# ziwang1121/IEEE

Measured on AMD Instinct MI355X. Metric: 3-modal images/s (train fwd+bwd), higher is better.
Workload: dtype bf16

## Files before the change

ieee_amd/csrc/bn.hip:

```cpp
#include <math.h>
#include <stdlib.h>

#include <hip/hip_ext.h>

#include <algorithm>
#include "common.h"
#include "pool_gather.h"

namespace ieee {

#ifndef IEEE_RED_MAX_BLOCKS
#define IEEE_RED_MAX_BLOCKS 768
#endif
constexpr int RED_MAX_BLOCKS = IEEE_RED_MAX_BLOCKS;

struct RedGeom {
  int M, C;
  int cprw;
  int tx, ty;
  int cblocks;
  int rblocks;
  int rows_per_block;
};

static RedGeom red_geom(int64_t M, int C, int vec) {
  RedGeom g;
  g.M = (int)M;
  g.C = C;
  g.cprw = C / vec;
  g.tx = g.cprw < 64 ? g.cprw : 64;
  int tx = 1;
  while (tx * 2 <= g.tx && g.cprw % (tx * 2) == 0) tx *= 2;
  g.tx = tx;
  g.ty = 256 / g.tx;
  g.cblocks = cdiv(g.cprw, g.tx);
  int rb = RED_MAX_BLOCKS / g.cblocks;
  if (rb < 1) rb = 1;
  const int maxrb = cdiv(M, g.ty * 4);
  if (rb > maxrb) rb = maxrb;
  if (rb < 1) rb = 1;
  g.rows_per_block = cdiv(cdiv(M, rb), g.ty) * g.ty;
  g.rblocks = cdiv(M, g.rows_per_block);
  return g;
}

template <typename T, int NQ, class F>
__device__ __forceinline__ void reduce_channels(const RedGeom& g, float* partial, int64_t partial_gs, F f) {
  constexpr int VEC = 16 / sizeof(T);
  __shared__ float red[256 * 8];
  const int t = threadIdx.x;
  const int tx = t % g.tx, ty = t / g.tx;
  const int cb = blockIdx.x % g.cblocks, rb = blockIdx.x / g.cblocks;
  const int chunk = cb * g.tx + tx;
  float acc[NQ][VEC];
#pragma unroll
  for (int q = 0; q < NQ; ++q)
#pragma unroll
    for (int e = 0; e < VEC; ++e) acc[q][e] = 0.f;
// ... 675 lines not shown
#pragma unroll
    for (int e = 0; e < VEC; ++e) {
      const float m = (v[e] * sc[c0 + e] + sh[c0 + e]) > 0.f ? d[e] : 0.f;
      acc[0][e] += m;
      acc[1][e] += m * v[e];
    }
  });
}

template <typename T>
__global__ __launch_bounds__(256) void bn_bwd_pooled_apply_kernel(const T* __restrict__ dpool,
                                                                  const uint8_t* __restrict__ arg,
                                                                  const T* __restrict__ y, T* __restrict__ dy,
                                                                  const float* __restrict__ coef, int64_t coef_gs,
                                                                  int64_t total_chunks, int cprw, int C, int64_t y_gs,
                                                                  int64_t p_gs, int Hi, int Wi, int Ho, int Wo,
                                                                  const float* __restrict__ stats, int64_t stats_gs,
                                                                  PoolShifts ps) {
  constexpr int VEC = 16 / sizeof(T);
  const int z = blockIdx.y;
  const float* sc = stats + z * stats_gs + 2 * C;
  const float* sh = sc + C;
  const float* k1 = coef + z * coef_gs;
  const float* k2 = k1 + C;
  const float* k3 = k2 + C;
  const T* dd = dpool + z * p_gs;
  const uint8_t* aa = arg + z * p_gs;
  const T* yy = y + z * y_gs;
  T* oo = dy + z * y_gs;
  const uint32_t total = (uint32_t)total_chunks, stride = gridDim.x * blockDim.x;
  for (uint32_t i = blockIdx.x * blockDim.x + threadIdx.x; i < total; i += stride) {
    int ch, row, w, h, b;
    if (ps.pow2) {
      ch = (int)(i & (uint32_t)(cprw - 1)); row = (int)(i >> ps.lq);
      w = row & (Wi - 1); h = (row >> ps.lw) & (Hi - 1); b = row >> (ps.lw + ps.lh);
    } else {
      ch = (int)(i % (uint32_t)cprw); row = (int)(i / (uint32_t)cprw);
      w = row % Wi; h = (row / Wi) % Hi; b = row / (Wi * Hi);
    }
    const int c0 = ch * VEC;
    float d[VEC], v[VEC];
    const uint4 yv = *(const uint4*)(yy + (int64_t)i * VEC);
    pool_grad_gather<T>(dd, aa, b, h, w, ch, Ho, Wo, C, d);
    Vec16<T>::unpack(yv, v);
#pragma unroll
    for (int e = 0; e < VEC; ++e) {
      const float m = (v[e] * sc[c0 + e] + sh[c0 + e]) > 0.f ? d[e] : 0.f;
      v[e] = k1[c0 + e] * m + k2[c0 + e] * v[e] + k3[c0 + e];
    }
    *(uint4*)(oo + (int64_t)i * VEC) = Vec16<T>::pack(v);
  }
}

template <typename T, bool APPLY>
__global__ __launch_bounds__(256) void bn_bwd_pooled_tiled_kernel(const T* __restrict__ dpool, const uint8_t* __restrict__ arg,
                                                                  const T* __restrict__ y, T* __restrict__ dy,
                                                                  const float* __restrict__ coef, int64_t coef_gs,
                                                                  float* __restrict__ partial, int64_t partial_gs, int C,
                                                                  int64_t y_gs, int64_t p_gs, int Hi, int Wi, int Ho, int Wo,
                                                                  const float* __restrict__ stats, int64_t stats_gs) {
  constexpr int VEC = 16 / sizeof(T);
  extern __shared__ __attribute__((aligned(16))) char pooled_lds[];
  const int z = blockIdx.y, t = threadIdx.x;
  const int hp = Hi >> 1;
  const int b = blockIdx.x / hp, p = blockIdx.x - b * hp;
  const int cprw = C / VEC, rowel = Wo * C;
  T* sd = (T*)pooled_lds;
  uint8_t* sa = (uint8_t*)(pooled_lds + 2 * rowel * sizeof(T));
  const bool has2 = p + 1 < Ho;
  {
    const int64_t o = z * p_gs + ((int64_t)b * Ho + p) * rowel;
    const uint4* dsrc = (const uint4*)(dpool + o);
    const uint4* asrc = (const uint4*)(arg + o);
    const int nd = (has2 ? 2 : 1) * rowel / VEC, na = (has2 ? 2 : 1) * rowel / 16;
    for (int i = t; i < nd; i += 256) ((uint4*)sd)[i] = dsrc[i];
    for (int i = t; i < na; i += 256) ((uint4*)sa)[i] = asrc[i];
  }
  __syncthreads();
  const float* sc = stats + z * stats_gs + 2 * C;
  const float* sh = sc + C;
  const float* k1 = coef + z * coef_gs;
  const float* k2 = k1 + C;
  const float* k3 = k2 + C;
  const T* yy = y + z * y_gs + (int64_t)b * Hi * Wi * C;
  T* oo = APPLY ? dy + z * y_gs + (int64_t)b * Hi * Wi * C : nullptr;
  const int ch = t % cprw, c0 = ch * VEC;
  float scl[VEC], shf[VEC], a1[VEC], a2[VEC], a3[VEC];
#pragma unroll
  for (int e = 0; e < VEC; ++e) {
    scl[e] = sc[c0 + e]; shf[e] = sh[c0 + e];
    if (APPLY) { a1[e] = k1[c0 + e]; a2[e] = k2[c0 + e]; a3[e] = k3[c0 + e]; } else { a1[e] = 0.f; a2[e] = 0.f; a3[e] = 0.f; }
  }
  float s1[VEC], s2[VEC];
#pragma unroll
  for (int e = 0; e < VEC; ++e) { s1[e] = 0.f; s2[e] = 0.f; }
  const int ppr = 256 / cprw;
  for (int px = t / cprw; px < 2 * Wi; px += ppr) {
    const int r = px >= Wi ? 1 : 0, w = px - r * Wi;
    const int q0 = w >> 1, lr0 = r + 1, lc0 = (w & 1) + 1;
    const bool c1 = (w & 1) && q0 + 1 < Wo, r1 = r == 1 && has2;
    const int64_t off = ((int64_t)(2 * p + r) * Wi + w) * C + c0;
    const uint4 yv = *(const uint4*)(yy + off);
    float d[VEC];
#pragma unroll
    for (int e = 0; e < VEC; ++e) d[e] = 0.f;
    auto window = [&](int lrow, int q, int local) {
      const int o = (lrow * Wo + q) * C + c0;
      float g[VEC];
      Vec16<T>::unpack(*(const uint4*)(sd + o), g);
      if constexpr (VEC == 8) {
        const uint2 av = *(const uint2*)(sa + o);
#pragma unroll
        for (int e = 0; e < 4; ++e) {
          if ((int)((av.x >> (8 * e)) & 0xff) == local) d[e] += g[e];
          if ((int)((av.y >> (8 * e)) & 0xff) == local) d[4 + e] += g[4 + e];
        }
      } else {
        const uint32_t av = *(const uint32_t*)(sa + o);
#pragma unroll
        for (int e = 0; e < VEC; ++e)
          if ((int)((av >> (8 * e)) & 0xff) == local) d[e] += g[e];
      }
    };
    window(0, q0, lr0 * 3 + lc0);
    if (c1) window(0, q0 + 1, lr0 * 3);
    if (r1) window(1, q0, lc0);
    if (r1 && c1) window(1, q0 + 1, 0);
    float v[VEC];
    Vec16<T>::unpack(yv, v);
#pragma unroll
    for (int e = 0; e < VEC; ++e) {
      const float m = (v[e] * scl[e] + shf[e]) > 0.f ? d[e] : 0.f;
      if (APPLY) {
        v[e] = a1[e] * m + a2[e] * v[e] + a3[e];
      } else {
        s1[e] += m;
        s2[e] += m * v[e];
      }
    }
    if (APPLY) *(uint4*)(oo + off) = Vec16<T>::pack(v);
  }
  if constexpr (!APPLY) {
    float* red = (float*)pooled_lds;
    float* out = partial + z * partial_gs + (int64_t)blockIdx.x * 2 * C;
#pragma unroll
    for (int qn = 0; qn < 2; ++qn) {
      __syncthreads();
#pragma unroll
      for (int e = 0; e < VEC; ++e) red[t * VEC + e] = qn == 0 ? s1[e] : s2[e];
      __syncthreads();
      for (int c = t; c < C; c += 256) {
        const int cc = c / VEC, e = c - cc * VEC;
        float s = 0.f;
        for (int k = cc; k < 256; k += cprw) s += red[k * VEC + e];
        out[qn * C + c] = s;
      }
    }
  }
}

static int tot_blocks(int64_t chunks, int64_t groups) {
  static const int64_t fixed = getenv("IEEE_BN_TOTALS_BLOCKS") ? atoll(getenv("IEEE_BN_TOTALS_BLOCKS")) : 0;
  const int64_t cap = fixed > 0 ? fixed : std::max<int64_t>(256, 2048 / std::max<int64_t>(groups, 1));
  int64_t b = (chunks + 255) / 256;
  if (b > cap) b = cap;
  if (b < 1) b = 1;
  return (int)b;
}

static int ew_blocks(int64_t chunks) {
  static const int64_t cap = getenv("IEEE_EW_BLOCKS") ? atoll(getenv("IEEE_EW_BLOCKS")) : 8192;
  int64_t b = (chunks + 255) / 256;
  if (b > cap) b = cap;
  if (b < 1) b = 1;
  return (int)b;
}

}

using namespace ieee;

static int vec_of(int dtype) { return dtype == IEEE_BF16 ? 8 : 4; }

static bool fixed_channel_ok(int which, int cprw, const void* p1, const void* p2) {
  static const int on = getenv("IEEE_BN_FIXED") ? atoi(getenv("IEEE_BN_FIXED")) : 8;
  return (on & which) && cprw >= 1 && cprw <= 256 && 256 % cprw == 0 && ((uintptr_t)p1 & 15) == 0 && ((uintptr_t)p2 & 15) == 0;
}
static int fixed_unroll() {
  static const int u = getenv("IEEE_BN_UNROLL") ? atoi(getenv("IEEE_BN_UNROLL")) : 1;
  return u == 2 ? 2 : 1;
}

extern "C" int64_t ieee_bn_partial_floats(int dtype, int64_t M, int64_t C) {
  const RedGeom g = red_geom(M, (int)C, vec_of(dtype));
  const int64_t rb = std::max((int64_t)g.rblocks, (M + 127) / 128);
  return rb * 2 * C;
}

extern "C" int ieee_bn2d_fwd(const void* y, const void* residual, void* out, int dtype, int64_t groups, int64_t M,
                             int64_t C, int64_t act_gs, const float* gamma, const float* beta, int64_t param_gs,
                             float* running_mean, float* running_var, int64_t buf_gs, float* stats, float* partial,
                             float momentum, float eps, int training, int relu, int64_t stats_rblocks, void* relu_bits,
                             void* stream) {
  IEEE_REQUIRE(y && gamma && beta && stats, "bn2d_fwd: null pointer");
  IEEE_REQUIRE(!relu_bits || (dtype == IEEE_BF16 && out && act_gs % 8 == 0), "bn2d_fwd: relu_bits needs a bf16 output");
  IEEE_REQUIRE(dtype == IEEE_F32 || dtype == IEEE_BF16, "bn2d_fwd: bad dtype");
  IEEE_REQUIRE(C % vec_of(dtype) == 0, "bn2d_fwd: C %ld not a multiple of %d", (long)C, vec_of(dtype));
  IEEE_REQUIRE(training || (running_mean && running_var), "bn2d_fwd: eval mode needs running stats");
  IEEE_REQUIRE(!training || partial, "bn2d_fwd: training needs the partial-sum scratch");
  hipStream_t st = (hipStream_t)stream;
  RedGeom g = red_geom(M, (int)C, vec_of(dtype));
// ... 252 lines not shown
                          (const bf16*)dout, (const bf16*)out_mask, (const bf16*)y, (bf16*)dy, (bf16*)g_out,                 \
                          (const long long*)totals, gamma, param_gs, stats, dgamma, dbeta, grad_gs, (int)M, chunks, cprw,    \
                          (int)C, act_gs, 1.0 / (double)M, replicas, groups * 2 * C, overflow);                              \
    break;
  switch (variant) {
    IEEE_BN_BWD_TOT(0, false) IEEE_BN_BWD_TOT(0, true) IEEE_BN_BWD_TOT(1, false) IEEE_BN_BWD_TOT(1, true)
    IEEE_BN_BWD_TOT(2, false) IEEE_BN_BWD_TOT(2, true)
  }
#undef IEEE_BN_BWD_TOT
  return launch_status("bn_bwd_apply_totals_kernel");
}

extern "C" int ieee_bn2d_bwd_totals_ds(const void* dout, const void* y, const void* y_ds, void* dy, int dtype, int64_t groups,
                                       int64_t M, int64_t C, int64_t act_gs, const float* gamma, int64_t param_gs,
                                       const float* stats, float* dgamma, float* dbeta, int64_t grad_gs, const void* totals,
                                       int replicas, void* totals_ds, int replicas_ds, int* overflow, void* done_event,
                                       void* stream) {
  IEEE_REQUIRE(replicas >= 1 && replicas <= 64 && replicas_ds >= 1 && replicas_ds <= 64, "bn2d_bwd_totals_ds: 1..64 replicas");
  IEEE_REQUIRE(dout && y && y_ds && dy && gamma && stats && totals && totals_ds, "bn2d_bwd_totals_ds: null pointer");
  IEEE_REQUIRE(dtype == IEEE_BF16, "bn2d_bwd_totals_ds: bf16 only");
  const int cprw = (int)(C / 8);
  IEEE_REQUIRE(C % 8 == 0 && cprw >= 1 && cprw <= 256 && 256 % cprw == 0, "bn2d_bwd_totals_ds: C / 8 must divide 256");
  IEEE_REQUIRE((((uintptr_t)totals | (uintptr_t)gamma | (uintptr_t)stats) & 15) == 0 && param_gs % 4 == 0,
               "bn2d_bwd_totals_ds: totals / gamma / stats must be 16-byte aligned (group stride a multiple of 4 floats)");
  hipStream_t st = (hipStream_t)stream;
  const int64_t chunks = M * C / 8;
  dim3 grid(tot_blocks(chunks, groups), (unsigned)groups);
  const size_t lds = std::max<size_t>(3 * C, 8 * 256) * sizeof(float);
  const float lim2 = nextafterf(4611686018427387904.0f / (float)grid.x, 0.f);
  hipExtLaunchKernelGGL((bn_bwd_apply_totals_ds_kernel<bf16>), grid, dim3(256), (uint32_t)lds, st, nullptr, (hipEvent_t)done_event, 0,
                        (const bf16*)dout, (const bf16*)y, (const bf16*)y_ds, (bf16*)dy, (const long long*)totals, gamma, param_gs,
                        stats, dgamma, dbeta, grad_gs, (int)M, chunks, cprw, (int)C, act_gs, 1.0 / (double)M, replicas,
                        groups * 2 * C, (long long*)totals_ds, replicas_ds, groups * 2 * C, lim2, overflow);
  return launch_status("bn_bwd_apply_totals_ds_kernel");
}

extern "C" int ieee_bn2d_bwd_pooled(const void* dpool, const uint8_t* argmax, const void* y, void* dy, int dtype,
                                    int64_t groups, int64_t B, int64_t Hi, int64_t Wi, int64_t C, const float* gamma,
                                    int64_t param_gs, const float* stats, float* dgamma, float* dbeta, int64_t grad_gs,
                                    float* partial, float* coef, int accumulate, void* stream) {
  IEEE_REQUIRE(dpool && argmax && y && dy && gamma && stats && partial && coef, "bn2d_bwd_pooled: null pointer");
  IEEE_REQUIRE(dtype == IEEE_F32 || dtype == IEEE_BF16, "bn2d_bwd_pooled: bad dtype");
  IEEE_REQUIRE(C % vec_of(dtype) == 0, "bn2d_bwd_pooled: C not a multiple of the vector width");
  IEEE_REQUIRE(B * Hi * Wi * C < (1ll << 31), "bn2d_bwd_pooled: more than 2^31 elements per group");
  hipStream_t st = (hipStream_t)stream;
  const int64_t M = B * Hi * Wi;
  const int Ho = (int)((Hi + 2 - 3) / 2 + 1), Wo = (int)((Wi + 2 - 3) / 2 + 1);
  const int64_t y_gs = M * C, p_gs = B * Ho * Wo * C;
  RedGeom g = red_geom(M, (int)C, vec_of(dtype));
  {
    static const bool tiled_on = !(getenv("IEEE_POOLED_TILED") && atoi(getenv("IEEE_POOLED_TILED")) == 0);
    const int vec = vec_of(dtype), es = dtype == IEEE_BF16 ? 2 : 4;
    const int64_t cprw = C / vec, rowel = (int64_t)Wo * C;
    const int64_t lds = std::max<int64_t>(2 * rowel * (es + 1), 256 * vec * 4);
    const int64_t rbt = B * (Hi / 2);
    if (tiled_on && Hi == 2 * Ho && Wi == 2 * Wo && Wi >= 64 && 256 % cprw == 0 && rowel % 16 == 0 && lds <= 64 * 1024 &&
        rbt <= (M + 127) / 128) {
      const int64_t partial_gs = rbt * 2 * C;
      dim3 tgrid((unsigned)rbt, (unsigned)groups);
      if (dtype == IEEE_F32)
        bn_bwd_pooled_tiled_kernel<float, false><<<tgrid, 256, lds, st>>>((const float*)dpool, argmax, (const float*)y, nullptr,
            coef, 3 * C, partial, partial_gs, (int)C, y_gs, p_gs, (int)Hi, (int)Wi, Ho, Wo, stats, 4 * C);
      else
        bn_bwd_pooled_tiled_kernel<bf16, false><<<tgrid, 256, lds, st>>>((const bf16*)dpool, argmax, (const bf16*)y, nullptr,
            coef, 3 * C, partial, partial_gs, (int)C, y_gs, p_gs, (int)Hi, (int)Wi, Ho, Wo, stats, 4 * C);
      IEEE_TRY(launch_status("bn_bwd_pooled_tiled_kernel(reduce)"));
      const int lpc = finalize_lpc(rbt);
      bn_bwd_finalize_kernel<<<dim3(cdiv(C, 256 / lpc), (unsigned)groups), 256, 0, st>>>(
          partial, partial_gs, (int)rbt, (int)M, (int)C, gamma, param_gs, stats, 4 * C, dgamma, dbeta, grad_gs, coef, 3 * C,
          accumulate, 0, lpc);
      IEEE_TRY(launch_status("bn_bwd_finalize_kernel"));
      if (dtype == IEEE_F32)
        bn_bwd_pooled_tiled_kernel<float, true><<<tgrid, 256, lds, st>>>((const float*)dpool, argmax, (const float*)y, (float*)dy,
            coef, 3 * C, nullptr, 0, (int)C, y_gs, p_gs, (int)Hi, (int)Wi, Ho, Wo, stats, 4 * C);
      else
        bn_bwd_pooled_tiled_kernel<bf16, true><<<tgrid, 256, lds, st>>>((const bf16*)dpool, argmax, (const bf16*)y, (bf16*)dy,
            coef, 3 * C, nullptr, 0, (int)C, y_gs, p_gs, (int)Hi, (int)Wi, Ho, Wo, stats, 4 * C);
      return launch_status("bn_bwd_pooled_tiled_kernel(apply)");
    }
  }
  const int64_t partial_gs = (int64_t)g.rblocks * 2 * C;
  dim3 rgrid(g.cblocks * g.rblocks, (unsigned)groups);
  auto lg = [](int64_t v) { int l = 0; while ((1ll << l) < v) ++l; return ((1ll << l) == v) ? l : -1; };
  PoolShifts ps;
  ps.lw = lg(Wi); ps.lh = lg(Hi); ps.lc = lg(C); ps.lq = lg(g.cprw);
  ps.pow2 = (ps.lw >= 0 && ps.lh >= 0 && ps.lc >= 0 && ps.lq >= 0) ? 1 : 0;
  if (dtype == IEEE_F32)
    bn_bwd_pooled_reduce_kernel<float><<<rgrid, 256, 0, st>>>((const float*)dpool, argmax, (const float*)y, y_gs, p_gs, g,
                                                              (int)Hi, (int)Wi, Ho, Wo, partial, partial_gs, stats, 4 * C, ps);
  else
    bn_bwd_pooled_reduce_kernel<bf16><<<rgrid, 256, 0, st>>>((const bf16*)dpool, argmax, (const bf16*)y, y_gs, p_gs, g,
                                                             (int)Hi, (int)Wi, Ho, Wo, partial, partial_gs, stats, 4 * C, ps);
  IEEE_TRY(launch_status("bn_bwd_pooled_reduce_kernel"));
  const int lpc = finalize_lpc(g.rblocks);
  bn_bwd_finalize_kernel<<<dim3(cdiv(C, 256 / lpc), (unsigned)groups), 256, 0, st>>>(
      partial, partial_gs, g.rblocks, (int)M, (int)C, gamma, param_gs, stats, 4 * C, dgamma, dbeta, grad_gs, coef,
      3 * C, accumulate, 0, lpc);
  IEEE_TRY(launch_status("bn_bwd_finalize_kernel"));
  const int64_t chunks = M * C / vec_of(dtype);
  dim3 grid(ew_blocks(chunks), (unsigned)groups);
  if (dtype == IEEE_F32)
    bn_bwd_pooled_apply_kernel<float><<<grid, 256, 0, st>>>((const float*)dpool, argmax, (const float*)y, (float*)dy, coef,
                                                            3 * C, chunks, g.cprw, (int)C, y_gs, p_gs, (int)Hi, (int)Wi, Ho,
                                                            Wo, stats, 4 * C, ps);
  else
    bn_bwd_pooled_apply_kernel<bf16><<<grid, 256, 0, st>>>((const bf16*)dpool, argmax, (const bf16*)y, (bf16*)dy, coef,
                                                           3 * C, chunks, g.cprw, (int)C, y_gs, p_gs, (int)Hi, (int)Wi, Ho,
                                                           Wo, stats, 4 * C, ps);
  return launch_status("bn_bwd_pooled_apply_kernel");
}
```

ieee_amd/csrc/cim.hip:

```cpp
#include <stdlib.h>

#include <type_traits>

#include "common.h"
#include "pool_gather.h"

namespace ieee {

template <typename T>
__global__ void nchw_to_nhwc_kernel(const float* x0, const float* x1, const float* x2, T* out, int B, int C, int H,
                                    int W, int Cpad, int pad) {
  const int z = blockIdx.y;
  const float* x = z == 0 ? x0 : (z == 1 ? x1 : x2);
  const int Hp = H + 2 * pad, Wp = W + 2 * pad;
  const int64_t total = (int64_t)B * Hp * Wp * Cpad;
  T* o = out + z * total;
  for (int64_t i = (int64_t)blockIdx.x * blockDim.x + threadIdx.x; i < total; i += (int64_t)gridDim.x * blockDim.x) {
    const int c = (int)(i % Cpad);
    int64_t p = i / Cpad;
    const int wp = (int)(p % Wp); p /= Wp;
    const int hp = (int)(p % Hp);
    const int b = (int)(p / Hp);
    const int h = hp - pad, w = wp - pad;
    float v = 0.f;
// ... 44 lines not shown
  out += z * o_gs;
  arg += z * o_gs;
  for (int i = blockIdx.x * blockDim.x + threadIdx.x; i < total; i += gridDim.x * blockDim.x) {
    int ch, q, pp, b;
    if (lq >= 0) {
      ch = i & (cprw - 1);
      const int p = i >> lq;
      q = p & (Wo - 1); pp = (p >> lw) & (Ho - 1); b = p >> (lw + lh);
    } else {
      ch = i % cprw;
      int p = i / cprw;
      q = p % Wo; p /= Wo;
      pp = p % Ho;
      b = p / Ho;
    }
    float best[VEC];
    int bi[VEC];
#pragma unroll
    for (int e = 0; e < VEC; ++e) { best[e] = -INFINITY; bi[e] = 0; }
#pragma unroll
    for (int r = 0; r < 3; ++r) {
      const int h = pp * 2 - 1 + r;
      if ((unsigned)h >= (unsigned)Hi) continue;
#pragma unroll
      for (int s = 0; s < 3; ++s) {
        const int w = q * 2 - 1 + s;
        if ((unsigned)w >= (unsigned)Wi) continue;
        float v[VEC];
        Vec16<T>::unpack(*(const uint4*)(x + (((int64_t)b * Hi + h) * Wi + w) * C + ch * VEC), v);
        if constexpr (AFFINE) {
#pragma unroll
          for (int e = 0; e < VEC; ++e) v[e] = fmaxf(v[e] * sc[ch * VEC + e] + sh[ch * VEC + e], 0.f);
          Vec16<T>::unpack(Vec16<T>::pack(v), v);
        }
#pragma unroll
        for (int e = 0; e < VEC; ++e)
          if (v[e] > best[e]) { best[e] = v[e]; bi[e] = r * 3 + s; }
      }
    }
    const int64_t o = (((int64_t)b * Ho + pp) * Wo + q) * C + ch * VEC;
    *(uint4*)(out + o) = Vec16<T>::pack(best);
    if constexpr (VEC == 8) {
      uint2 pk = make_uint2(0u, 0u);
#pragma unroll
      for (int e = 0; e < 4; ++e) { pk.x |= (unsigned)bi[e] << (8 * e); pk.y |= (unsigned)bi[4 + e] << (8 * e); }
      *(uint2*)(arg + o) = pk;
    } else {
#pragma unroll
      for (int e = 0; e < VEC; ++e) arg[o + e] = (uint8_t)bi[e];
    }
  }
}

template <typename T>
__global__ __launch_bounds__(256) void bn_relu_maxpool_tiled_kernel(const T* __restrict__ y, T* __restrict__ out,
                                                                    uint8_t* __restrict__ arg, int Hi, int Wi, int C, int Ho,
                                                                    int Wo, int64_t x_gs, int64_t o_gs,
                                                                    const float* __restrict__ stats, int64_t stats_gs) {
  constexpr int VEC = 16 / sizeof(T);
  extern __shared__ __attribute__((aligned(16))) char pool_lds[];
  T* sa = (T*)pool_lds;
  const int z = blockIdx.y, t = threadIdx.x;
  const int b = blockIdx.x / Ho, p = blockIdx.x - b * Ho;
  const int cprw = C / VEC, rowch = Wi * cprw;
  const float* sc = stats + z * stats_gs + 2 * C;
  const float* sh = sc + C;
  const T* yy = y + z * x_gs + (int64_t)b * Hi * Wi * C;
  for (int idx = t; idx < 3 * rowch; idx += 256) {
    const int r = idx / rowch, rem = idx - r * rowch;
    const int h = 2 * p - 1 + r;
    if ((unsigned)h >= (unsigned)Hi) continue;
    const int c0 = (rem % cprw) * VEC;
    float v[VEC];
    Vec16<T>::unpack(*(const uint4*)(yy + ((int64_t)h * Wi) * C + (int64_t)rem * VEC), v);
#pragma unroll
    for (int e = 0; e < VEC; ++e) v[e] = fmaxf(v[e] * sc[c0 + e] + sh[c0 + e], 0.f);
    *(uint4*)(sa + (int64_t)idx * VEC) = Vec16<T>::pack(v);
  }
  __syncthreads();
  for (int idx = t; idx < Wo * cprw; idx += 256) {
    const int q = idx / cprw, ch = idx - q * cprw;
    float best[VEC];
    int bi[VEC];
#pragma unroll
    for (int e = 0; e < VEC; ++e) { best[e] = -INFINITY; bi[e] = 0; }
#pragma unroll
    for (int r = 0; r < 3; ++r) {
      const int h = 2 * p - 1 + r;
      if ((unsigned)h >= (unsigned)Hi) continue;
#pragma unroll
      for (int s2 = 0; s2 < 3; ++s2) {
        const int w = q * 2 - 1 + s2;
        if ((unsigned)w >= (unsigned)Wi) continue;
        float v[VEC];
        Vec16<T>::unpack(*(const uint4*)(sa + ((int64_t)(r * Wi + w) * cprw + ch) * VEC), v);
#pragma unroll
        for (int e = 0; e < VEC; ++e)
          if (v[e] > best[e]) { best[e] = v[e]; bi[e] = r * 3 + s2; }
      }
    }
    const int64_t o = z * o_gs + (((int64_t)b * Ho + p) * Wo + q) * C + ch * VEC;
    *(uint4*)(out + o) = Vec16<T>::pack(best);
    if constexpr (VEC == 8) {
      uint2 pk = make_uint2(0u, 0u);
#pragma unroll
      for (int e = 0; e < 4; ++e) { pk.x |= (unsigned)bi[e] << (8 * e); pk.y |= (unsigned)bi[4 + e] << (8 * e); }
      *(uint2*)(arg + o) = pk;
    } else {
#pragma unroll
      for (int e = 0; e < VEC; ++e) arg[o + e] = (uint8_t)bi[e];
    }
  }
}

template <typename T>
__global__ __launch_bounds__(256) void maxpool_bwd_kernel(const T* __restrict__ dout, const uint8_t* __restrict__ arg,
                                                          T* __restrict__ dx, int B, int Hi, int Wi, int C, int Ho,
                                                          int Wo, int64_t x_gs, int64_t o_gs) {
  constexpr int VEC = 16 / sizeof(T);
  const int z = blockIdx.y;
  const int cprw = C / VEC;
  const int total = B * Hi * Wi * cprw;
  dout += z * o_gs;
  arg += z * o_gs;
  dx += z * x_gs;
  for (int i = blockIdx.x * blockDim.x + threadIdx.x; i < total; i += gridDim.x * blockDim.x) {
    const int ch = i % cprw;
    int p = i / cprw;
    const int w = p % Wi; p /= Wi;
    const int h = p % Hi;
    const int b = p / Hi;
    float acc[VEC];
    pool_grad_gather<T>(dout, arg, b, h, w, ch, Ho, Wo, C, acc);
    *(uint4*)(dx + i * VEC) = Vec16<T>::pack(acc);
  }
}

struct PosGeom {
  int B, P, C;
  int W;
  int cprw, tx, ty, cblocks;
};
static PosGeom pos_geom(int B, int H, int W, int C, int vec) {
  PosGeom g;
  g.B = B; g.P = H * W; g.C = C; g.W = W;
  g.cprw = C / vec;
  int tx = 1;
  while (tx * 2 <= 64 && g.cprw % (tx * 2) == 0) tx *= 2;
  g.tx = tx;
  g.ty = 256 / tx;
  g.cblocks = g.cprw / tx;
  return g;
}

__device__ __forceinline__ int bin_start(int i, int H, int parts) { return (i * H) / parts; }
__device__ __forceinline__ int bin_end(int i, int H, int parts) { return ((i + 1) * H + parts - 1) / parts; }

constexpr int RED_Q = 8;
template <int NQV>
__device__ __forceinline__ void reduce_over_ty(float* acc, int tx, int ty, int txn, int tyn, float* red) {
#pragma unroll
  for (int q0 = 0; q0 < NQV; q0 += RED_Q) {
    __syncthreads();
#pragma unroll
    for (int q = 0; q < RED_Q; ++q)
// ... 469 lines not shown
  do {                                                              \
    if ((dtype) == IEEE_F32) { CALL_F32; }                          \
    else if ((dtype) == IEEE_BF16) { CALL_BF16; }                   \
    else { IEEE_REQUIRE(false, "bad dtype %d", (int)(dtype)); }     \
  } while (0)

extern "C" int ieee_nchw_to_nhwc3(const float* x_rgb, const float* x_ni, const float* x_ti, void* out, int dtype,
                                  int64_t B, int64_t C, int64_t H, int64_t W, int64_t Cpad, int64_t pad, void* stream) {
  IEEE_REQUIRE(x_rgb && x_ni && x_ti && out, "nchw_to_nhwc3: null pointer");
  IEEE_REQUIRE(Cpad >= C && pad >= 0, "nchw_to_nhwc3: Cpad < C or negative padding");
  hipStream_t st = (hipStream_t)stream;
  if (dtype == IEEE_BF16 && Cpad == 4 && C <= 4 && ((W + 2 * pad) & 1) == 0 &&
      B * (H + 2 * pad) * (W + 2 * pad) < (1ll << 30)) {
    dim3 grid2(ew_blocks2(B * (H + 2 * pad) * ((W + 2 * pad) / 2)), 3);
    nchw_to_nhwc4_bf16_kernel<<<grid2, 256, 0, st>>>(x_rgb, x_ni, x_ti, (bf16*)out, (int)B, (int)C, (int)H, (int)W, (int)pad);
    return launch_status("nchw_to_nhwc4_bf16_kernel");
  }
  dim3 grid(ew_blocks2(B * Cpad * (H + 2 * pad) * (W + 2 * pad)), 3);
  DISPATCH_T(dtype, (nchw_to_nhwc_kernel<float><<<grid, 256, 0, st>>>(x_rgb, x_ni, x_ti, (float*)out, (int)B, (int)C, (int)H, (int)W, (int)Cpad, (int)pad)),
             (nchw_to_nhwc_kernel<bf16><<<grid, 256, 0, st>>>(x_rgb, x_ni, x_ti, (bf16*)out, (int)B, (int)C, (int)H, (int)W, (int)Cpad, (int)pad)));
  return launch_status("nchw_to_nhwc_kernel");
}

extern "C" int ieee_maxpool3x3s2_fwd(const void* x, void* out, uint8_t* argmax, int dtype, int64_t groups, int64_t B,
                                     int64_t Hi, int64_t Wi, int64_t C, void* stream) {
  IEEE_REQUIRE(x && out && argmax, "maxpool_fwd: null pointer");
  IEEE_REQUIRE(C % vecw(dtype) == 0, "maxpool_fwd: C not a multiple of the vector width");
  IEEE_REQUIRE(B * Hi * Wi * C < (1ll << 31), "maxpool_fwd: more than 2^31 elements per group");
  const int Ho = (int)((Hi + 2 - 3) / 2 + 1), Wo = (int)((Wi + 2 - 3) / 2 + 1);
  hipStream_t st = (hipStream_t)stream;
  dim3 grid(ew_blocks2(B * Ho * Wo * C / vecw(dtype)), (unsigned)groups);
  const int64_t xgs = B * Hi * Wi * C, ogs = B * Ho * Wo * C;
  auto lg = [](int64_t v) { int l = 0; while ((1ll << l) < v) ++l; return ((1ll << l) == v) ? l : -1; };
  int lq = lg(C / vecw(dtype)), lw = lg(Wo), lh = lg(Ho);
  if (lq < 0 || lw < 0 || lh < 0) lq = -1;
  DISPATCH_T(dtype, (maxpool_fwd_kernel<float, false><<<grid, 256, 0, st>>>((const float*)x, (float*)out, argmax, (int)B, (int)Hi, (int)Wi, (int)C, Ho, Wo, xgs, ogs, lq, lw, lh, nullptr, 0)),
             (maxpool_fwd_kernel<bf16, false><<<grid, 256, 0, st>>>((const bf16*)x, (bf16*)out, argmax, (int)B, (int)Hi, (int)Wi, (int)C, Ho, Wo, xgs, ogs, lq, lw, lh, nullptr, 0)));
  return launch_status("maxpool_fwd_kernel");
}

extern "C" int ieee_bn_relu_maxpool3x3s2_fwd(const void* y, const float* stats, void* out, uint8_t* argmax, int dtype,
                                             int64_t groups, int64_t B, int64_t Hi, int64_t Wi, int64_t C, void* stream) {
  IEEE_REQUIRE(y && stats && out && argmax, "bn_relu_maxpool_fwd: null pointer");
  IEEE_REQUIRE(C % vecw(dtype) == 0, "bn_relu_maxpool_fwd: C not a multiple of the vector width");
  IEEE_REQUIRE(B * Hi * Wi * C < (1ll << 31), "bn_relu_maxpool_fwd: more than 2^31 elements per group");
  const int Ho = (int)((Hi + 2 - 3) / 2 + 1), Wo = (int)((Wi + 2 - 3) / 2 + 1);
  hipStream_t st = (hipStream_t)stream;
  dim3 grid(ew_blocks2(B * Ho * Wo * C / vecw(dtype)), (unsigned)groups);
  const int64_t xgs = B * Hi * Wi * C, ogs = B * Ho * Wo * C;
  {
    static const bool tiled_on = !(getenv("IEEE_POOL_TILED") && atoi(getenv("IEEE_POOL_TILED")) == 0);
    const int64_t lds = 3 * Wi * C * (dtype == IEEE_BF16 ? 2 : 4);
    if (tiled_on && lds <= 64 * 1024 && Wi >= 32) {
      dim3 tgrid((unsigned)(B * Ho), (unsigned)groups);
      DISPATCH_T(dtype, (bn_relu_maxpool_tiled_kernel<float><<<tgrid, 256, lds, st>>>((const float*)y, (float*)out, argmax, (int)Hi, (int)Wi, (int)C, Ho, Wo, xgs, ogs, stats, 4 * C)),
                 (bn_relu_maxpool_tiled_kernel<bf16><<<tgrid, 256, lds, st>>>((const bf16*)y, (bf16*)out, argmax, (int)Hi, (int)Wi, (int)C, Ho, Wo, xgs, ogs, stats, 4 * C)));
      return launch_status("bn_relu_maxpool_tiled_kernel");
    }
  }
  auto lg = [](int64_t v) { int l = 0; while ((1ll << l) < v) ++l; return ((1ll << l) == v) ? l : -1; };
  int lq = lg(C / vecw(dtype)), lw = lg(Wo), lh = lg(Ho);
  if (lq < 0 || lw < 0 || lh < 0) lq = -1;
  DISPATCH_T(dtype, (maxpool_fwd_kernel<float, true><<<grid, 256, 0, st>>>((const float*)y, (float*)out, argmax, (int)B, (int)Hi, (int)Wi, (int)C, Ho, Wo, xgs, ogs, lq, lw, lh, stats, 4 * C)),
             (maxpool_fwd_kernel<bf16, true><<<grid, 256, 0, st>>>((const bf16*)y, (bf16*)out, argmax, (int)B, (int)Hi, (int)Wi, (int)C, Ho, Wo, xgs, ogs, lq, lw, lh, stats, 4 * C)));
  return launch_status("maxpool_fwd_kernel(affine)");
}

extern "C" int ieee_maxpool3x3s2_bwd(const void* dout, const uint8_t* argmax, void* dx, int dtype, int64_t groups,
                                     int64_t B, int64_t Hi, int64_t Wi, int64_t C, void* stream) {
  IEEE_REQUIRE(dout && dx && argmax, "maxpool_bwd: null pointer");
  IEEE_REQUIRE(B * Hi * Wi * C < (1ll << 31), "maxpool_bwd: more than 2^31 elements per group");
  const int Ho = (int)((Hi + 2 - 3) / 2 + 1), Wo = (int)((Wi + 2 - 3) / 2 + 1);
  hipStream_t st = (hipStream_t)stream;
  dim3 grid(ew_blocks2(B * Hi * Wi * C / vecw(dtype)), (unsigned)groups);
  const int64_t xgs = B * Hi * Wi * C, ogs = B * Ho * Wo * C;
  DISPATCH_T(dtype, (maxpool_bwd_kernel<float><<<grid, 256, 0, st>>>((const float*)dout, argmax, (float*)dx, (int)B, (int)Hi, (int)Wi, (int)C, Ho, Wo, xgs, ogs)),
             (maxpool_bwd_kernel<bf16><<<grid, 256, 0, st>>>((const bf16*)dout, argmax, (bf16*)dx, (int)B, (int)Hi, (int)Wi, (int)C, Ho, Wo, xgs, ogs)));
  return launch_status("maxpool_bwd_kernel");
}

extern "C" int ieee_gpool_sum_others(const void* F, void* S, float* Gp, int dtype, int64_t B, int64_t H, int64_t W,
                                     int64_t C, void* stream) {
  IEEE_REQUIRE(F && Gp, "gpool_sum_others: null pointer");
  IEEE_REQUIRE(C % (vecw(dtype)) == 0, "gpool_sum_others: bad C");
  const PosGeom g = pos_geom((int)B, (int)H, (int)W, (int)C, vecw(dtype));
  hipStream_t st = (hipStream_t)stream;
  const int64_t gs = B * H * W * C;
  dim3 grid((unsigned)(B * g.cblocks));
  DISPATCH_T(dtype, (gpool_sum_others_kernel<float><<<grid, 256, 0, st>>>((const float*)F, (float*)S, Gp, g, gs, S ? 1 : 0)),
             (gpool_sum_others_kernel<bf16><<<grid, 256, 0, st>>>((const bf16*)F, (bf16*)S, Gp, g, gs, S ? 1 : 0)));
  return launch_status("gpool_sum_others_kernel");
}

extern "C" int ieee_ca_pool(const void* y2, const float* stats2, float* avg, float* mx, int64_t pool_gs,
                            int32_t* argmax, int dtype, int64_t B, int64_t H, int64_t W, int64_t C, void* stream) {
  IEEE_REQUIRE(y2 && stats2 && avg && mx && argmax, "ca_pool: null pointer");
  const PosGeom g = pos_geom((int)B, (int)H, (int)W, (int)C, vecw(dtype));
  hipStream_t st = (hipStream_t)stream;
  dim3 grid((unsigned)(B * g.cblocks), 3);
  DISPATCH_T(dtype, (ca_pool_kernel<float><<<grid, 256, 0, st>>>((const float*)y2, stats2, avg, mx, argmax, g, B * H * W * C, pool_gs)),
             (ca_pool_kernel<bf16><<<grid, 256, 0, st>>>((const bf16*)y2, stats2, avg, mx, argmax, g, B * H * W * C, pool_gs)));
  return launch_status("ca_pool_kernel");
}

extern "C" int ieee_cim_tail_fwd(const void* y1, const void* y2, const float* stats1, const float* stats2,
                                 const float* att, float* parts_out, int dtype, int64_t B, int64_t H, int64_t W,
                                 int64_t C, int64_t parts, int mode, void* stream) {
  IEEE_REQUIRE(y1 && parts_out, "cim_tail_fwd: null pointer");
  IEEE_REQUIRE(parts >= 1 && parts <= 8, "cim_tail_fwd: parts must be in [1,8]");
// ... 67 lines not shown
```

Before: 4462.

## Walk multiple pooled rows per block with rolling LDS ring and prefetch

Both the fused BN+ReLU+maxpool forward kernel and the pooled BN backward kernel now have each block walk a run of consecutive output rows instead of handling one row. A 3-row LDS ring buffer keeps overlapping rows resident, and the next row's inputs are prefetched into registers while the current row is processed. This cuts redundant global reloads of shared halo rows and reduces the number of blocks and per-block setup. The backward reduction also switches to a padded transposed LDS layout that sums both statistics in one pass. The cost is fewer blocks, so less parallelism, plus more registers, inline asm moves, and a heuristic walk length.

```diff
diff --git a/ieee_amd/csrc/bn.hip b/ieee_amd/csrc/bn.hip
--- a/ieee_amd/csrc/bn.hip
+++ b/ieee_amd/csrc/bn.hip
@@ -4,6 +4,7 @@
 #include <hip/hip_ext.h>
 
 #include <algorithm>
+#include <type_traits>
 #include "common.h"
 #include "pool_gather.h"
 
@@ -785,31 +786,26 @@
   }
 }
 
+constexpr int POOLED_PY = 4;
 template <typename T, bool APPLY>
 __global__ __launch_bounds__(256) void bn_bwd_pooled_tiled_kernel(const T* __restrict__ dpool, const uint8_t* __restrict__ arg,
                                                                   const T* __restrict__ y, T* __restrict__ dy,
                                                                   const float* __restrict__ coef, int64_t coef_gs,
                                                                   float* __restrict__ partial, int64_t partial_gs, int C,
                                                                   int64_t y_gs, int64_t p_gs, int Hi, int Wi, int Ho, int Wo,
-                                                                  const float* __restrict__ stats, int64_t stats_gs) {
+                                                                  const float* __restrict__ stats, int64_t stats_gs, int walk,
+                                                                  int runs) {
   constexpr int VEC = 16 / sizeof(T);
   extern __shared__ __attribute__((aligned(16))) char pooled_lds[];
   const int z = blockIdx.y, t = threadIdx.x;
-  const int hp = Hi >> 1;
-  const int b = blockIdx.x / hp, p = blockIdx.x - b * hp;
+  const int b = blockIdx.x / runs, run = blockIdx.x - b * runs;
+  const int pa = run * walk, pe = min(Ho, pa + walk);
   const int cprw = C / VEC, rowel = Wo * C;
+  const int nd = rowel / VEC, na = rowel / 16;
   T* sd = (T*)pooled_lds;
-  uint8_t* sa = (uint8_t*)(pooled_lds + 2 * rowel * sizeof(T));
-  const bool has2 = p + 1 < Ho;
-  {
-    const int64_t o = z * p_gs + ((int64_t)b * Ho + p) * rowel;
-    const uint4* dsrc = (const uint4*)(dpool + o);
-    const uint4* asrc = (const uint4*)(arg + o);
-    const int nd = (has2 ? 2 : 1) * rowel / VEC, na = (has2 ? 2 : 1) * rowel / 16;
-    for (int i = t; i < nd; i += 256) ((uint4*)sd)[i] = dsrc[i];
-    for (int i = t; i < na; i += 256) ((uint4*)sa)[i] = asrc[i];
-  }
-  __syncthreads();
+  uint8_t* sa = (uint8_t*)(pooled_lds + 3 * rowel * sizeof(T));
+  const T* dimg = dpool + z * p_gs + (int64_t)b * Ho * rowel;
+  const uint8_t* aimg = arg + z * p_gs + (int64_t)b * Ho * rowel;
   const float* sc = stats + z * stats_gs + 2 * C;
   const float* sh = sc + C;
   const float* k1 = coef + z * coef_gs;
@@ -818,6 +814,21 @@
   const T* yy = y + z * y_gs + (int64_t)b * Hi * Wi * C;
   T* oo = APPLY ? dy + z * y_gs + (int64_t)b * Hi * Wi * C : nullptr;
   const int ch = t % cprw, c0 = ch * VEC;
+  const int ppr = 256 / cprw, px0 = t / cprw;
+  for (int r = pa; r < min(Ho, pa + 2); ++r) {
+    const uint4* dsrc = (const uint4*)(dimg + (int64_t)r * rowel);
+    const uint4* asrc = (const uint4*)(aimg + (int64_t)r * rowel);
+    uint4* dd = (uint4*)(sd + (r % 3) * rowel);
+    uint4* ad = (uint4*)(sa + (r % 3) * rowel);
+    for (int i = t; i < nd; i += 256) dd[i] = dsrc[i];
+    for (int i = t; i < na; i += 256) ad[i] = asrc[i];
+  }
+  uint4 yn[POOLED_PY];
+#pragma unroll
+  for (int j = 0; j < POOLED_PY; ++j) {
+    const int px = px0 + j * ppr;
+    yn[j] = px < 2 * Wi ? *(const uint4*)(yy + ((int64_t)2 * pa * Wi + px) * C + c0) : make_uint4(0u, 0u, 0u, 0u);
+  }
   float scl[VEC], shf[VEC], a1[VEC], a2[VEC], a3[VEC];
 #pragma unroll
   for (int e = 0; e < VEC; ++e) {
@@ -827,69 +838,116 @@
   float s1[VEC], s2[VEC];
 #pragma unroll
   for (int e = 0; e < VEC; ++e) { s1[e] = 0.f; s2[e] = 0.f; }
-  const int ppr = 256 / cprw;
-  for (int px = t / cprw; px < 2 * Wi; px += ppr) {
-    const int r = px >= Wi ? 1 : 0, w = px - r * Wi;
-    const int q0 = w >> 1, lr0 = r + 1, lc0 = (w & 1) + 1;
-    const bool c1 = (w & 1) && q0 + 1 < Wo, r1 = r == 1 && has2;
-    const int64_t off = ((int64_t)(2 * p + r) * Wi + w) * C + c0;
-    const uint4 yv = *(const uint4*)(yy + off);
-    float d[VEC];
-#pragma unroll
-    for (int e = 0; e < VEC; ++e) d[e] = 0.f;
-    auto window = [&](int lrow, int q, int local) {
-      const int o = (lrow * Wo + q) * C + c0;
-      float g[VEC];
-      Vec16<T>::unpack(*(const uint4*)(sd + o), g);
-      if constexpr (VEC == 8) {
-        const uint2 av = *(const uint2*)(sa + o);
-#pragma unroll
-        for (int e = 0; e < 4; ++e) {
-          if ((int)((av.x >> (8 * e)) & 0xff) == local) d[e] += g[e];
-          if ((int)((av.y >> (8 * e)) & 0xff) == local) d[4 + e] += g[4 + e];
+  __syncthreads();
+  auto pair = [&](const int p, auto more_c) {
+    constexpr bool more = decltype(more_c)::value;
+    const bool has2 = p + 1 < Ho;
+    const bool newrow = more && p + 2 < Ho;
+    uint4 dn = make_uint4(0u, 0u, 0u, 0u), an = dn;
+    const uint4* dsrc = (const uint4*)(dimg + (int64_t)(p + 2) * rowel);
+    const uint4* asrc = (const uint4*)(aimg + (int64_t)(p + 2) * rowel);
+    if (newrow) {
+      if (t < nd) dn = dsrc[t];
+      if (t < na) an = asrc[t];
+    }
+    const T* sd0 = sd + (p % 3) * rowel;
+    const T* sd1 = sd + ((p + 1) % 3) * rowel;
+    const uint8_t* sa0 = sa + (p % 3) * rowel;
+    const uint8_t* sa1 = sa + ((p + 1) % 3) * rowel;
+    auto pixel = [&](int px, const uint4 yv) {
+      const int r = px >= Wi ? 1 : 0, w = px - r * Wi;
+      const int q0 = w >> 1, lr0 = r + 1, lc0 = (w & 1) + 1;
+      const bool c1 = (w & 1) && q0 + 1 < Wo, r1 = r == 1 && has2;
+      float d[VEC];
+#pragma unroll
+      for (int e = 0; e < VEC; ++e) d[e] = 0.f;
+      auto window = [&](const T* srow, const uint8_t* arow, int q, int local) {
+        const int o = q * C + c0;
+        float g[VEC];
+        Vec16<T>::unpack(*(const uint4*)(srow + o), g);
+        if constexpr (VEC == 8) {
+          const uint2 av = *(const uint2*)(arow + o);
+#pragma unroll
+          for (int e = 0; e < 4; ++e) {
+            if ((int)((av.x >> (8 * e)) & 0xff) == local) d[e] += g[e];
+            if ((int)((av.y >> (8 * e)) & 0xff) == local) d[4 + e] += g[4 + e];
+          }
+        } else {
+          const uint32_t av = *(const uint32_t*)(arow + o);
+#pragma unroll
+          for (int e = 0; e < VEC; ++e)
+            if ((int)((av >> (8 * e)) & 0xff) == local) d[e] += g[e];
         }
-      } else {
-        const uint32_t av = *(const uint32_t*)(sa + o);
-#pragma unroll
-        for (int e = 0; e < VEC; ++e)
-          if ((int)((av >> (8 * e)) & 0xff) == local) d[e] += g[e];
+      };
+      window(sd0, sa0, q0, lr0 * 3 + lc0);
+      if (c1) window(sd0, sa0, q0 + 1, lr0 * 3);
+      if (r1) window(sd1, sa1, q0, lc0);
+      if (r1 && c1) window(sd1, sa1, q0 + 1, 0);
+      float v[VEC];
+      Vec16<T>::unpack(yv, v);
+#pragma unroll
+      for (int e = 0; e < VEC; ++e) {
+        const float m = (v[e] * scl[e] + shf[e]) > 0.f ? d[e] : 0.f;
+        if (APPLY) {
+          v[e] = a1[e] * m + a2[e] * v[e] + a3[e];
+        } else {
+          s1[e] += m;
+          s2[e] += m * v[e];
+        }
       }
+      if (APPLY) *(uint4*)(oo + ((int64_t)2 * p * Wi + px) * C + c0) = Vec16<T>::pack(v);
     };
-    window(0, q0, lr0 * 3 + lc0);
-    if (c1) window(0, q0 + 1, lr0 * 3);
-    if (r1) window(1, q0, lc0);
-    if (r1 && c1) window(1, q0 + 1, 0);
-    float v[VEC];
-    Vec16<T>::unpack(yv, v);
-#pragma unroll
-    for (int e = 0; e < VEC; ++e) {
-      const float m = (v[e] * scl[e] + shf[e]) > 0.f ? d[e] : 0.f;
-      if (APPLY) {
-        v[e] = a1[e] * m + a2[e] * v[e] + a3[e];
-      } else {
-        s1[e] += m;
-        s2[e] += m * v[e];
-      }
-    }
-    if (APPLY) *(uint4*)(oo + off) = Vec16<T>::pack(v);
-  }
+#pragma unroll
+    for (int j = 0; j < POOLED_PY; ++j) {
+      int px = px0 + j * ppr;
+      asm volatile("" : "+v"(px));
+      uint4 yv;
+      asm volatile("v_mov_b32 %0, %1" : "=v"(yv.x) : "v"(yn[j].x));
+      asm volatile("v_mov_b32 %0, %1" : "=v"(yv.y) : "v"(yn[j].y));
+      asm volatile("v_mov_b32 %0, %1" : "=v"(yv.z) : "v"(yn[j].z));
+      asm volatile("v_mov_b32 %0, %1" : "=v"(yv.w) : "v"(yn[j].w));
+      if constexpr (more) yn[j] = *(const uint4*)(yy + ((int64_t)2 * (p + 1) * Wi + min(px, 2 * Wi - 1)) * C + c0);
+      if (px < 2 * Wi) pixel(px, yv);
+    }
+    for (int px = px0 + POOLED_PY * ppr; px < 2 * Wi; px += ppr)
+      pixel(px, *(const uint4*)(yy + ((int64_t)2 * p * Wi + px) * C + c0));
+    if (newrow) {
+      uint4* dd = (uint4*)(sd + ((p + 2) % 3) * rowel);
+      uint4* ad = (uint4*)(sa + ((p + 2) % 3) * rowel);
+      if (t < nd) dd[t] = dn;
+      if (t < na) ad[t] = an;
+      for (int i = t + 256; i < nd; i += 256) dd[i] = dsrc[i];
+      for (int i = t + 256; i < na; i += 256) ad[i] = asrc[i];
+    }
+    __syncthreads();
+  };
+  for (int p = pa; p + 1 < pe; ++p) pair(p, std::true_type());
+  pair(pe - 1, std::false_type());
   if constexpr (!APPLY) {
     float* red = (float*)pooled_lds;
     float* out = partial + z * partial_gs + (int64_t)blockIdx.x * 2 * C;
 #pragma unroll
-    for (int qn = 0; qn < 2; ++qn) {
-      __syncthreads();
-#pragma unroll
-      for (int e = 0; e < VEC; ++e) red[t * VEC + e] = qn == 0 ? s1[e] : s2[e];
-      __syncthreads();
-      for (int c = t; c < C; c += 256) {
-        const int cc = c / VEC, e = c - cc * VEC;
-        float s = 0.f;
-        for (int k = cc; k < 256; k += cprw) s += red[k * VEC + e];
-        out[qn * C + c] = s;
-      }
-    }
-  }
+    for (int e = 0; e < VEC; ++e) { red[e * 257 + t] = s1[e]; red[(VEC + e) * 257 + t] = s2[e]; }
+    __syncthreads();
+    for (int i = t; i < 2 * C; i += 256) {
+      const int qn = i >= C ? 1 : 0, c = i - qn * C;
+      const int cc = c / VEC, e = c - cc * VEC;
+      const float* src = red + (qn * VEC + e) * 257;
+      float s = 0.f;
+      for (int k = cc; k < 256; k += cprw) s += src[k];
+      out[qn * C + c] = s;
+    }
+  }
+}
+
+static int walk_len(int forced, int64_t units, int64_t images, int64_t groups) {
+  if (forced > 0) return (int)std::min<int64_t>(forced, units);
+  const int64_t cap = std::max<int64_t>(256, 2048 / std::max<int64_t>(groups, 1));
+  const int64_t rpi = std::min(units, std::max<int64_t>(1, cap / std::max<int64_t>(images, 1)));
+  const int64_t w0 = (units + rpi - 1) / rpi;
+  for (int64_t w = w0; w < 2 * w0 && w <= units; ++w)
+    if (units % w == 0) return (int)w;
+  return (int)w0;
 }
 
 static int tot_blocks(int64_t chunks, int64_t groups) {
@@ -1248,18 +1306,21 @@
     static const bool tiled_on = !(getenv("IEEE_POOLED_TILED") && atoi(getenv("IEEE_POOLED_TILED")) == 0);
     const int vec = vec_of(dtype), es = dtype == IEEE_BF16 ? 2 : 4;
     const int64_t cprw = C / vec, rowel = (int64_t)Wo * C;
-    const int64_t lds = std::max<int64_t>(2 * rowel * (es + 1), 256 * vec * 4);
-    const int64_t rbt = B * (Hi / 2);
+    const int64_t lds = std::max<int64_t>(3 * rowel * (es + 1), 2 * 257 * vec * 4);
     if (tiled_on && Hi == 2 * Ho && Wi == 2 * Wo && Wi >= 64 && 256 % cprw == 0 && rowel % 16 == 0 && lds <= 64 * 1024 &&
-        rbt <= (M + 127) / 128) {
+        B * (Hi / 2) <= (M + 127) / 128) {
+      const char* wenv = getenv("IEEE_POOLED_WALK");
+      const int walk = walk_len(wenv ? atoi(wenv) : 0, Hi / 2, B, groups);
+      const int runs = cdiv(Hi / 2, walk);
+      const int64_t rbt = B * runs;
       const int64_t partial_gs = rbt * 2 * C;
       dim3 tgrid((unsigned)rbt, (unsigned)groups);
       if (dtype == IEEE_F32)
         bn_bwd_pooled_tiled_kernel<float, false><<<tgrid, 256, lds, st>>>((const float*)dpool, argmax, (const float*)y, nullptr,
-            coef, 3 * C, partial, partial_gs, (int)C, y_gs, p_gs, (int)Hi, (int)Wi, Ho, Wo, stats, 4 * C);
+            coef, 3 * C, partial, partial_gs, (int)C, y_gs, p_gs, (int)Hi, (int)Wi, Ho, Wo, stats, 4 * C, walk, runs);
       else
         bn_bwd_pooled_tiled_kernel<bf16, false><<<tgrid, 256, lds, st>>>((const bf16*)dpool, argmax, (const bf16*)y, nullptr,
-            coef, 3 * C, partial, partial_gs, (int)C, y_gs, p_gs, (int)Hi, (int)Wi, Ho, Wo, stats, 4 * C);
+            coef, 3 * C, partial, partial_gs, (int)C, y_gs, p_gs, (int)Hi, (int)Wi, Ho, Wo, stats, 4 * C, walk, runs);
       IEEE_TRY(launch_status("bn_bwd_pooled_tiled_kernel(reduce)"));
       const int lpc = finalize_lpc(rbt);
       bn_bwd_finalize_kernel<<<dim3(cdiv(C, 256 / lpc), (unsigned)groups), 256, 0, st>>>(
@@ -1268,10 +1329,10 @@
       IEEE_TRY(launch_status("bn_bwd_finalize_kernel"));
       if (dtype == IEEE_F32)
         bn_bwd_pooled_tiled_kernel<float, true><<<tgrid, 256, lds, st>>>((const float*)dpool, argmax, (const float*)y, (float*)dy,
-            coef, 3 * C, nullptr, 0, (int)C, y_gs, p_gs, (int)Hi, (int)Wi, Ho, Wo, stats, 4 * C);
+            coef, 3 * C, nullptr, 0, (int)C, y_gs, p_gs, (int)Hi, (int)Wi, Ho, Wo, stats, 4 * C, walk, runs);
       else
         bn_bwd_pooled_tiled_kernel<bf16, true><<<tgrid, 256, lds, st>>>((const bf16*)dpool, argmax, (const bf16*)y, (bf16*)dy,
-            coef, 3 * C, nullptr, 0, (int)C, y_gs, p_gs, (int)Hi, (int)Wi, Ho, Wo, stats, 4 * C);
+            coef, 3 * C, nullptr, 0, (int)C, y_gs, p_gs, (int)Hi, (int)Wi, Ho, Wo, stats, 4 * C, walk, runs);
       return launch_status("bn_bwd_pooled_tiled_kernel(apply)");
     }
   }
diff --git a/ieee_amd/csrc/cim.hip b/ieee_amd/csrc/cim.hip
--- a/ieee_amd/csrc/cim.hip
+++ b/ieee_amd/csrc/cim.hip
@@ -120,65 +120,118 @@
   }
 }
 
+constexpr int POOL_PF = 4;
 template <typename T>
 __global__ __launch_bounds__(256) void bn_relu_maxpool_tiled_kernel(const T* __restrict__ y, T* __restrict__ out,
                                                                     uint8_t* __restrict__ arg, int Hi, int Wi, int C, int Ho,
                                                                     int Wo, int64_t x_gs, int64_t o_gs,
-                                                                    const float* __restrict__ stats, int64_t stats_gs) {
+                                                                    const float* __restrict__ stats, int64_t stats_gs, int walk,
+                                                                    int runs) {
   constexpr int VEC = 16 / sizeof(T);
   extern __shared__ __attribute__((aligned(16))) char pool_lds[];
   T* sa = (T*)pool_lds;
   const int z = blockIdx.y, t = threadIdx.x;
-  const int b = blockIdx.x / Ho, p = blockIdx.x - b * Ho;
+  const int b = blockIdx.x / runs, run = blockIdx.x - b * runs;
+  const int pa = run * walk, pe = min(Ho, pa + walk);
   const int cprw = C / VEC, rowch = Wi * cprw;
   const float* sc = stats + z * stats_gs + 2 * C;
   const float* sh = sc + C;
   const T* yy = y + z * x_gs + (int64_t)b * Hi * Wi * C;
+  const bool fixed = 256 % cprw == 0;
+  float scl[VEC], shf[VEC];
+#pragma unroll
+  for (int e = 0; e < VEC; ++e) {
+    scl[e] = fixed ? sc[(t % cprw) * VEC + e] : 0.f;
+    shf[e] = fixed ? sh[(t % cprw) * VEC + e] : 0.f;
+  }
+  auto put = [&](int h, int rem, const uint4 raw) {
+    float v[VEC];
+    Vec16<T>::unpack(raw, v);
+    if (fixed) {
+#pragma unroll
+      for (int e = 0; e < VEC; ++e) v[e] = fmaxf(v[e] * scl[e] + shf[e], 0.f);
+    } else {
+      const int c0 = (rem % cprw) * VEC;
+#pragma unroll
+      for (int e = 0; e < VEC; ++e) v[e] = fmaxf(v[e] * sc[c0 + e] + sh[c0 + e], 0.f);
+    }
+    *(uint4*)(sa + ((int64_t)((h + 1) % 3) * rowch + rem) * VEC) = Vec16<T>::pack(v);
+  };
   for (int idx = t; idx < 3 * rowch; idx += 256) {
     const int r = idx / rowch, rem = idx - r * rowch;
-    const int h = 2 * p - 1 + r;
+    const int h = 2 * pa - 1 + r;
     if ((unsigned)h >= (unsigned)Hi) continue;
-    const int c0 = (rem % cprw) * VEC;
-    float v[VEC];
-    Vec16<T>::unpack(*(const uint4*)(yy + ((int64_t)h * Wi) * C + (int64_t)rem * VEC), v);
-#pragma unroll
-    for (int e = 0; e < VEC; ++e) v[e] = fmaxf(v[e] * sc[c0 + e] + sh[c0 + e], 0.f);
-    *(uint4*)(sa + (int64_t)idx * VEC) = Vec16<T>::pack(v);
+    put(h, rem, *(const uint4*)(yy + ((int64_t)h * Wi) * C + (int64_t)rem * VEC));
   }
   __syncthreads();
-  for (int idx = t; idx < Wo * cprw; idx += 256) {
-    const int q = idx / cprw, ch = idx - q * cprw;
-    float best[VEC];
-    int bi[VEC];
-#pragma unroll
-    for (int e = 0; e < VEC; ++e) { best[e] = -INFINITY; bi[e] = 0; }
-#pragma unroll
-    for (int r = 0; r < 3; ++r) {
-      const int h = 2 * p - 1 + r;
-      if ((unsigned)h >= (unsigned)Hi) continue;
-#pragma unroll
-      for (int s2 = 0; s2 < 3; ++s2) {
-        const int w = q * 2 - 1 + s2;
-        if ((unsigned)w >= (unsigned)Wi) continue;
-        float v[VEC];
-        Vec16<T>::unpack(*(const uint4*)(sa + ((int64_t)(r * Wi + w) * cprw + ch) * VEC), v);
-#pragma unroll
-        for (int e = 0; e < VEC; ++e)
-          if (v[e] > best[e]) { best[e] = v[e]; bi[e] = r * 3 + s2; }
-      }
-    }
-    const int64_t o = z * o_gs + (((int64_t)b * Ho + p) * Wo + q) * C + ch * VEC;
-    *(uint4*)(out + o) = Vec16<T>::pack(best);
-    if constexpr (VEC == 8) {
-      uint2 pk = make_uint2(0u, 0u);
-#pragma unroll
-      for (int e = 0; e < 4; ++e) { pk.x |= (unsigned)bi[e] << (8 * e); pk.y |= (unsigned)bi[4 + e] << (8 * e); }
-      *(uint2*)(arg + o) = pk;
-    } else {
-#pragma unroll
-      for (int e = 0; e < VEC; ++e) arg[o + e] = (uint8_t)bi[e];
-    }
-  }
+  for (int p = pa; p < pe; ++p) {
+    const int h0 = 2 * p + 2;
+    const int nnew = p + 1 < pe ? (min(Hi, h0 + 2) - h0) * rowch : 0;
+    const uint4* src = (const uint4*)(yy + (int64_t)h0 * Wi * C);
+    uint4 pre[POOL_PF];
+#pragma unroll
+    for (int j = 0; j < POOL_PF; ++j) {
+      const int i = t + j * 256;
+      pre[j] = i < nnew ? src[i] : make_uint4(0u, 0u, 0u, 0u);
+    }
+    auto scan = [&](const int idx) {
+      const int q = idx / cprw, ch = idx - q * cprw;
+      float best[VEC];
+      int bi[VEC];
+#pragma unroll
+      for (int e = 0; e < VEC; ++e) { best[e] = -INFINITY; bi[e] = 0; }
+#pragma unroll
+      for (int r = 0; r < 3; ++r) {
+        const int h = 2 * p - 1 + r;
+        if ((unsigned)h >= (unsigned)Hi) continue;
+        const T* srow = sa + (int64_t)((h + 1) % 3) * rowch * VEC;
+#pragma unroll
+        for (int s2 = 0; s2 < 3; ++s2) {
+          const int w = q * 2 - 1 + s2;
+          if ((unsigned)w >= (unsigned)Wi) continue;
+          float v[VEC];
+          Vec16<T>::unpack(*(const uint4*)(srow + ((int64_t)w * cprw + ch) * VEC), v);
+#pragma unroll
+          for (int e = 0; e < VEC; ++e)
+            if (v[e] > best[e]) { best[e] = v[e]; bi[e] = r * 3 + s2; }
+        }
+      }
+      const int64_t o = z * o_gs + (((int64_t)b * Ho + p) * Wo + q) * C + ch * VEC;
+      *(uint4*)(out + o) = Vec16<T>::pack(best);
+      if constexpr (VEC == 8) {
+        uint2 pk = make_uint2(0u, 0u);
+#pragma unroll
+        for (int e = 0; e < 4; ++e) { pk.x |= (unsigned)bi[e] << (8 * e); pk.y |= (unsigned)bi[4 + e] << (8 * e); }
+        *(uint2*)(arg + o) = pk;
+      } else {
+#pragma unroll
+        for (int e = 0; e < VEC; ++e) arg[o + e] = (uint8_t)bi[e];
+      }
+    };
+    if (t < Wo * cprw) scan(t);
+    for (int idx = t + 256; idx < Wo * cprw; idx += 256) scan(idx);
+    if (nnew == 0) break;
+    __syncthreads();
+#pragma unroll
+    for (int j = 0; j < POOL_PF; ++j) {
+      const int i = t + j * 256;
+      if (i < nnew) put(h0 + (i >= rowch ? 1 : 0), i >= rowch ? i - rowch : i, pre[j]);
+    }
+    for (int i = t + POOL_PF * 256; i < nnew; i += 256) put(h0 + (i >= rowch ? 1 : 0), i >= rowch ? i - rowch : i, src[i]);
+    __syncthreads();
+  }
+}
+
+static int pool_walk_len(int forced, int64_t units, int64_t images, int64_t groups) {
+  if (forced > 0) return (int)(forced < units ? forced : units);
+  const int64_t cap = 2048 / (groups > 1 ? groups : 1) > 256 ? 2048 / (groups > 1 ? groups : 1) : 256;
+  int64_t rpi = cap / (images > 1 ? images : 1);
+  if (rpi < 1) rpi = 1;
+  if (rpi > units) rpi = units;
+  const int64_t w0 = (units + rpi - 1) / rpi;
+  for (int64_t w = w0; w < 2 * w0 && w <= units; ++w)
+    if (units % w == 0) return (int)w;
+  return (int)w0;
 }
 
 template <typename T>
@@ -754,9 +807,12 @@
     static const bool tiled_on = !(getenv("IEEE_POOL_TILED") && atoi(getenv("IEEE_POOL_TILED")) == 0);
     const int64_t lds = 3 * Wi * C * (dtype == IEEE_BF16 ? 2 : 4);
     if (tiled_on && lds <= 64 * 1024 && Wi >= 32) {
-      dim3 tgrid((unsigned)(B * Ho), (unsigned)groups);
-      DISPATCH_T(dtype, (bn_relu_maxpool_tiled_kernel<float><<<tgrid, 256, lds, st>>>((const float*)y, (float*)out, argmax, (int)Hi, (int)Wi, (int)C, Ho, Wo, xgs, ogs, stats, 4 * C)),
-                 (bn_relu_maxpool_tiled_kernel<bf16><<<tgrid, 256, lds, st>>>((const bf16*)y, (bf16*)out, argmax, (int)Hi, (int)Wi, (int)C, Ho, Wo, xgs, ogs, stats, 4 * C)));
+      const char* wenv = getenv("IEEE_POOL_WALK");
+      const int walk = pool_walk_len(wenv ? atoi(wenv) : 0, Ho, B, groups);
+      const int runs = (Ho + walk - 1) / walk;
+      dim3 tgrid((unsigned)(B * runs), (unsigned)groups);
+      DISPATCH_T(dtype, (bn_relu_maxpool_tiled_kernel<float><<<tgrid, 256, lds, st>>>((const float*)y, (float*)out, argmax, (int)Hi, (int)Wi, (int)C, Ho, Wo, xgs, ogs, stats, 4 * C, walk, runs)),
+                 (bn_relu_maxpool_tiled_kernel<bf16><<<tgrid, 256, lds, st>>>((const bf16*)y, (bf16*)out, argmax, (int)Hi, (int)Wi, (int)C, Ho, Wo, xgs, ogs, stats, 4 * C, walk, runs)));
       return launch_status("bn_relu_maxpool_tiled_kernel");
     }
   }
```

Result: slower. 4406 (-1.3%).
